# HENDRIX-ZT2/pyaudiorestoration

Measured on AMD Instinct MI355X. Metric: Msamples/sec resampled (192 kHz varispeed), higher is better.
Workload: dtype f32 near taps, far taps (|n| >= 3) as float16 hi + lo x 2^-12 filter banks on v_mfma_f32_16x16x32_f16 with f32 accumulation / f64 positions

## Files before the change

pyaudiorestoration_amd/csrc/pos.hip:

```cpp
#include "par_common.h"
#include "pos_plan.h"
#include <math.h>
#include <vector>

#pragma clang fp contract(off)

namespace par {

struct AddU128 {
  using T = U128;
  __device__ static T identity() { return T{0ull, 0ull}; }
  __device__ static T combine(T a, T b) {
    T r;
    r.lo = a.lo + b.lo;
    r.hi = a.hi + b.hi + (r.lo < a.lo ? 1ull : 0ull);
    return r;
  }
};
struct AddF64 {
  using T = double;
  __device__ static T identity() { return 0.0; }
  __device__ static T combine(T a, T b) { return a + b; }
};
struct ComposeP {
// ... 869 lines not shown
  if (x < n_tiles) {
    const long long start = seg_start[lo], k = sample - start, b = k >> 3;
    static_assert(kCk == 8, "k >> 3");
    const double off = seg_off[lo];
    const bool off_ok = fabs(off) < 4.0e18;
    const double ro = off_ok ? rint(off) : 0.0;
    const long long slot = ck_slot0(start, lo) + b;
    const double ckv = lazy ? (lazy_segment_ok(seg_start[lo + 1] - start, sp[lo], sp[lo + 1])
                                   ? lazy_prefix(sp[lo], (sp[lo + 1] - sp[lo]) / (double)(seg_start[lo + 1] - start - 1), (double)(k + 1))
                                   : 0.0)
                            : ((b && slot < ck_len) ? ck[slot] : 0.0);
    const double rel = (off_ok ? off - ro : 0.0) + ckv;
    const bool ok = off_ok && fabs(rel) < 1.0e15 && ro > -0x1p61 && ro < 0x1p61;
    TileHdr hd;
    hd.anchor = ok ? ((long long)ro + (long long)rint(rel)) & ~1ll : 0ll;
    hd.c_last = 0;
    hd.iT = lo;
    hd.mn_rel = 0;
    bool may_unity = false, may_slow = false;
    for (long long q = lo; q < nseg && seg_start[q] <= sample + kSincTileOutputs; ++q) {
      may_unity = may_unity || !(sp[q] < kUnityHintBelow) || !(sp[q + 1] < kUnityHintBelow);
      may_slow = may_slow || !(sp[q] >= kSlowHintBelow) || !(sp[q + 1] >= kSlowHintBelow);
    }
    hd.flags = (ok ? 0 : 1) | (may_unity ? kTileMayUnity : 0) | (may_slow ? kTileMaySlow : 0) | (lazy ? kTileLazy : 0);
    hdr[x] = hd;
  }
}

__device__ __forceinline__ void tile_seg_body(const double* __restrict__ sp, const int64_t* __restrict__ seg_start,
                           const double* __restrict__ seg_off, int64_t nseg, const double* __restrict__ ck, int64_t ck_len,
                           int64_t max_tiles, int64_t* __restrict__ tile_seg, SegFast* __restrict__ seg_fast,
                           long long* __restrict__ tile_st, TileHdr* __restrict__ hdr, PlanHeader* __restrict__ h, const int64_t x,
                           const bool lazy = false) {
// ... 92 lines not shown
  const double z = rc * step;
  double cprev = ckv;
  if (uk) {
    if (fast) {
      const double x = z * (-0.5 * (double)(uk + 1) - 16.0);
      const double r = rc * __builtin_fma(x, __builtin_fma(x, -x, x) - 1.0, 1.0);
      cprev += r * (double)uk * __builtin_fma(z * z, (double)(uk * uk - 1) * (1.0 / 12.0), 1.0);
    } else {
      for (int v = 0; v < uk; ++v) cprev += recip_nr(__builtin_fma(step, k - (double)(uk - v), s0));
    }
  }
  return piece_poly(foff + cprev, rc, z, -16);
}
__device__ __forceinline__ bool irel_ok(long long rel) { return rel > -32000 && rel < 32000; }

__global__ __launch_bounds__(256) void k_block_rec2(const double* __restrict__ sp, const int64_t* __restrict__ seg_start,
                                                    int64_t nseg, const SegFast* __restrict__ seg_fast,
                                                    const TileHdr* __restrict__ hdr, BlockRec* __restrict__ rec,
                                                    BlockRec2* __restrict__ rec2, const PlanHeader* __restrict__ h) {
  const long long i = (long long)blockIdx.x * blockDim.x + threadIdx.x;
  if (i < 1 || i >= nseg || !h->ck_valid) return;
  const long long start = seg_start[i];
  const int us = (int)(start & (kRec - 1));
  if (us == 0 || start >= h->len_out) return;
  const SegFast s1 = seg_fast[i];
  const double rc = recip_nr(__builtin_fma(s1.step, (double)(16 - us), sp[i]));
  const BlockPoly b1 = piece_poly(s1.foff, rc, rc * s1.step, us - 16);
  const double r1 = rint(b1.a0);
  const long long rel = s1.A + (long long)r1 - hdr[start / kSincTileOutputs].anchor;
  BlockRec2 o2;
  o2.w0 = (unsigned)((int)rel << 16);
  o2.F = (float)(b1.a0 - r1);
  o2.e1 = (float)b1.a1m1;
  o2.e2 = (float)b1.a2;
  rec2[start >> kRecShift] = o2;
  if (!(fabs(b1.a0) < 1.0e9 && irel_ok(rel))) atomicOr(&rec[start >> kRecShift].w0, kRecSlow1);
}

__global__ __launch_bounds__(256) void k_block_rec(const double* __restrict__ sp, const int64_t* __restrict__ seg_start,
                                                   int64_t nseg, const double* __restrict__ ck,
                                                   const int64_t* __restrict__ tile_seg, const long long* __restrict__ tile_st,
                                                   const SegFast* __restrict__ seg_fast, const TileHdr* __restrict__ hdr,
                                                   BlockRec* __restrict__ rec, const PlanHeader* __restrict__ h) {
  const long long len_out = h->len_out;
  if (!h->ck_valid) return;
  const long long g = (long long)blockIdx.x * blockDim.x + threadIdx.x;
  const long long jb = g * kRec;
  if (jb >= len_out) return;
  const long long T = g / kBlocksPerTile;
  const long long j0 = T * kSincTileOutputs;
  const long long iT = tile_seg[T];
  int Sr[kTileStarts];
#pragma unroll
  for (int q = 0; q < kTileStarts; ++q) {
    const long long d = tile_st[T * kTileStarts + q] - j0;
    Sr[q] = d < -0x40000000ll ? -0x40000000 : (d > 0x40000000ll ? 0x40000000 : (int)d);
  }
// ... 60 lines not shown
    end1 = s1.n == need;
    slow1 = !(i + 1 < nseg && s1.fast >= 2 && s1.n >= need && s1.A > -(1ll << 61) && s1.A < (1ll << 61) && sp1 >= 0.971 &&
              sp1 <= 1.031) ||
            (ul >= (long long)ustar && ul < kRec);
    cubic |= s1.fast == 2;
  }
  BlockRec o;
  const bool e0 = (ustar < (unsigned)kRec) || rem == kRec;
  if (end1) slow1 = 1u;
  o.w0 = ((unsigned)((int)rel0 << 16)) | (ustar - 1u) | (e0 ? kRecE0 : 0u) | (end1 ? kRecE1 : 0u) | (slow0 ? kRecSlow0 : 0u) |
         (slow1 ? kRecSlow1 : 0u) | (cubic ? kRecCubic : 0u) | ((e0 ? ustar - 1u : 63u) << kRecLastShift);
  o.F = (float)(q0.a0 - r0);
  o.e1 = (float)q0.a1m1;
  o.e2 = (float)q0.a2;
  rec[g] = o;
}

constexpr int kRecLazySegs = 64;
#ifndef PAR_REC_EXP
#define PAR_REC_EXP 0
#endif
__device__ __forceinline__ double recip_nr_c(double b) {
#pragma clang fp contract(fast)
  double x = __builtin_amdgcn_rcp(b);
  x = x + x * (1.0 - b * x);
  return x + x * (1.0 - b * x);
}
__device__ __forceinline__ BlockPoly piece_poly_c(double base, double rc, double z, int d0) {
#pragma clang fp contract(fast)
  const double rp = -(rc * z), cz = rc * z * z, dd0 = (double)d0;
  const double s2m = (dd0 - 1.0) * dd0 * (2.0 * dd0 - 1.0) * (1.0 / 6.0);
  BlockPoly q;
  q.a0 = ((base + rc * (1.0 - dd0)) + 0.5 * rp * (dd0 - dd0 * dd0)) - cz * s2m;
  q.a1m1 = ((rc - 1.0) + 0.5 * rp) + cz * (1.0 / 6.0);
  q.a2 = 0.5 * rp + 0.5 * cz;
  return q;
}
__device__ __forceinline__ double lazy_prefix_nr(double s0, double step, double K) {
#pragma clang fp contract(fast)
  const double rc = recip_nr_c(__builtin_fma(step, 0.5 * (K - 1.0), s0));
  const double z = rc * step, t = z * z, K2 = K * K;
  return K * rc * (1.0 + t * (K2 - 1.0) * (1.0 / 12.0) * (1.0 + t * (3.0 * K2 - 7.0) * 0.05));
}
__global__ __launch_bounds__(256) void k_block_rec_lazy(const double* __restrict__ sp, const int64_t* __restrict__ seg_start,
                                                        int64_t nseg, const SegFast* __restrict__ seg_fast,
                                                        const TileHdr* __restrict__ hdr, BlockRec* __restrict__ rec,
                                                        BlockRec2* __restrict__ rec2, const PlanHeader* __restrict__ h) {
  __shared__ SegFast s_sf[4][kRecLazySegs + 1];
  __shared__ double s_sp[4][kRecLazySegs + 2];
  __shared__ int s_a[4][kRecLazySegs + 1];
  __shared__ unsigned char s_fl[4][kRecLazySegs];
  __shared__ unsigned char s_seg[4][kRecLazySegs * (kLazyMaxN / kRec)];
  static_assert(kLazyMaxN % kRec == 0 && kRecLazySegs <= 256, "a segment owns <= kLazyMaxN / kRec block starts; indices fit a byte");
  constexpr unsigned kF_Slow1 = 1u, kF_End1 = 2u, kF_Cubic1 = 4u;
  if (h->ck_valid != 2) return;
  const int l = threadIdx.x & (kWave - 1), w = threadIdx.x >> 6;
  const long long i0 = ((long long)blockIdx.x * 4 + w) * kRecLazySegs;
  if (i0 >= nseg) return;
  const long long len_out = h->len_out;
  const long long a0 = seg_start[i0];
  if (a0 >= len_out) return;
// ... 105 lines not shown
    o.F = (float)(q0.a0 - r0);
    o.e1 = (float)q0.a1m1;
    o.e2 = (float)q0.a2;
#if PAR_REC_EXP & 1
    if (o.w0 == 0x12345678u)
#endif
#if PAR_REC_EXP & 4
    {
      typedef unsigned u4v __attribute__((ext_vector_type(4)));
      u4v v = {o.w0, __float_as_uint(o.F), __float_as_uint(o.e1), __float_as_uint(o.e2)};
      __builtin_nontemporal_store(v, reinterpret_cast<u4v*>(rec + g));
    }
#else
    rec[g] = o;
#endif
  }
}

__device__ __forceinline__ void mark_direct(long long i, long long* direct, PlanHeader* h) {
  const int slot = atomicAdd(&h->n_direct, 1);
  if (slot < kMaxDirect) direct[slot] = i;
  else atomicOr(&h->flags, kFlagDirectOverflow);
}

__global__ void k_off_prepare(const double* __restrict__ S, const double* __restrict__ xs, const double* __restrict__ st,
                              int64_t nseg, PElem* __restrict__ el, long long* __restrict__ direct,
                              PlanHeader* __restrict__ h) {
  const int64_t i = (int64_t)blockIdx.x * blockDim.x + threadIdx.x;
  if (i >= nseg) return;
  const double st0 = st[0];
// ... 751 lines not shown
  hipLaunchKernelGGL(k_long_map, dim3(gc), dim3(256), 0, s, speeds, pv.seg_start, nseg, ck, ck_len, G, pv.hdr);
  hipLaunchKernelGGL(k_long_wmap, dim3(gw), dim3(256), 0, s, pv.seg_start, nseg, ck, ck_len, GW, pv.hdr);
  hipLaunchKernelGGL(k_long_stitch, dim3(gs), dim3(256), 0, s, speeds, pv.seg_start, nseg, ck, ck_len, pv.hdr);
  hipLaunchKernelGGL(k_long_wapply, dim3(gw), dim3(256), 0, s, pv.seg_start, nseg, ck, ck_len, GW, pv.hdr);
  hipLaunchKernelGGL(k_long_final, dim3(gc), dim3(256), 0, s, speeds, pv.seg_start, nseg, pv.S, ck, ck_len, G, pv.hdr);
  return PAR_OK;
}

static void launch_block_rec(const double* speeds, const par::PlanView& pv, int64_t nseg, void* aux, int64_t max_out, int64_t m,
                             hipStream_t s) {
  using namespace par;
  const FusedAux a = fused_aux_view(aux, max_out, m);
  const int64_t blocks = (int64_t)fused_blocks(max_out);
  hipLaunchKernelGGL(k_block_rec, dim3((unsigned)ceil_div(blocks, 256)), dim3(256), 0, s, speeds, pv.seg_start, nseg,
                     (const double*)a.ck, (const int64_t*)a.tile_seg, (const long long*)a.tile_st, (const SegFast*)a.seg_fast,
                     (const TileHdr*)a.hdr, a.rec, (const PlanHeader*)pv.hdr);
  hipLaunchKernelGGL(k_block_rec2, dim3((unsigned)ceil_div(nseg, 256)), dim3(256), 0, s, speeds, pv.seg_start, nseg,
                     (const SegFast*)a.seg_fast, (const TileHdr*)a.hdr, a.rec, a.rec2, (const PlanHeader*)pv.hdr);
}

static thread_local int g_last_plan_flags = 0;

static int plan_impl(int device, const double* sampletimes, const double* speeds, int64_t m, int64_t n_in, void* work,
                     size_t work_bytes, void* aux, size_t aux_bytes, int64_t max_out, int64_t* len_out, int* trimmed,
                     int force_host, int* path_used, int* fused_ok, void* stream) {
  using namespace par;
  PAR_REQUIRE(sampletimes && speeds && work && len_out && trimmed, PAR_ERR_ARG, "par_speed_to_pos_plan: null pointer");
  PAR_REQUIRE(m >= 2, PAR_ERR_ARG, "par_speed_to_pos_plan: need at least 2 speed samples (m=%lld)", (long long)m);
  PAR_REQUIRE(work_bytes >= plan_bytes(m), PAR_ERR_WORKSPACE, "par_speed_to_pos_plan: workspace %zu < %zu", work_bytes,
              plan_bytes(m));
  PAR_REQUIRE(!aux || aux_bytes >= fused_aux_bytes(max_out, m), PAR_ERR_WORKSPACE,
              "par_speed_to_pos_plan: aux buffer %zu < %zu", aux_bytes, aux ? fused_aux_bytes(max_out, m) : (size_t)0);
  PAR_HIP_CHECK(hipSetDevice(device));
// ... 54 lines not shown
    hipLaunchKernelGGL(k_off_heads, dim3((kMaxDirect + 255) / 256), dim3(256), 0, s, el, nseg, pv.direct, pv.hdr);
    hipLaunchKernelGGL(k_scan_reduce<ComposeP>, dim3(nbs), dim3(kScanThreads), 0, s, (const PElem*)el, nseg,
                       reinterpret_cast<PElem*>(pv.bsum));
    hipLaunchKernelGGL(k_scan_top<ComposeP>, dim3(1), dim3(kScanThreads), 0, s, reinterpret_cast<PElem*>(pv.bsum), (int64_t)nbs);
    hipLaunchKernelGGL(k_scan_apply<ComposeP>, dim3(nbs), dim3(kScanThreads), 0, s, el, nseg, (const PElem*)pv.bsum);
    hipLaunchKernelGGL(k_off_stitch, dim3(1), dim3(1), 0, s, pv.S, el, sampletimes, nseg, pv.direct, pv.runs, pv.hdr);
    if (lazy) {
      hipLaunchKernelGGL(k_off_apply, dim3(g256), dim3(256), 0, s, speeds, (const PElem*)el, (const RunEntry*)pv.runs, nseg,
                         (double)n_in, pv.seg_off, pv.hdr);
      hipLaunchKernelGGL(k_trim_lazy, dim3(1), dim3(1), 0, s, sampletimes, speeds, (const int64_t*)pv.seg_start,
                         (const double*)pv.seg_off, m, (double)n_in, ck_len, max_tiles, pv.hdr);
      const FusedAux av = fused_aux_view(aux, max_out, m);
      hipLaunchKernelGGL(k_tile_seg_lazy, dim3(g256), dim3(256), 0, s, speeds, (const int64_t*)pv.seg_start,
                         (const double*)pv.seg_off, nseg, av.tile_seg, av.seg_fast, av.tile_st, av.hdr, (const PlanHeader*)pv.hdr);
      hipLaunchKernelGGL(k_block_rec_lazy, dim3((unsigned)ceil_div(nseg, 4 * kRecLazySegs)), dim3(256), 0, s, speeds, (const int64_t*)pv.seg_start, nseg,
                         (const SegFast*)av.seg_fast, (const TileHdr*)av.hdr, av.rec, av.rec2, (const PlanHeader*)pv.hdr);
    } else {
    hipLaunchKernelGGL(k_off_apply_trim, dim3(g256 < 512u ? g256 : 512u), dim3(256), 0, s, sampletimes, speeds, (const PElem*)el,
                       (const RunEntry*)pv.runs, (const int64_t*)pv.seg_start, nseg, (double)n_in, pv.seg_off,
                       (const double*)ck, ck_len, pv.hdr);
    }
    if (aux && !lazy) {
      const int64_t n_items = std::max<int64_t>(nseg, max_tiles);
      hipLaunchKernelGGL(k_tile_seg_publish, dim3((unsigned)std::min<int64_t>(ceil_div(n_items, 256), 512)), dim3(256), 0, s,
                         speeds, pv.seg_start, pv.seg_off, nseg, (const double*)ck, ck_len, max_tiles,
                         reinterpret_cast<int64_t*>(ck + ck_len), reinterpret_cast<SegFast*>(ck + ck_len + max_tiles),
                         fused_aux_view(aux, max_out, m).tile_st, fused_aux_view(aux, max_out, m).hdr, pv.hdr, n_items,
                         lazy ? 1 : 0);
      launch_block_rec(speeds, pv, nseg, aux, max_out, m, s);
    }
    PAR_HIP_CHECK(hipGetLastError());
// ... 110 lines not shown
```

pyaudiorestoration_amd/csrc/pos_plan.h:

```cpp
#pragma once
#include "par_common.h"

namespace par {

struct PlanHeader {
  int64_t m;
  int64_t len_out;
  int64_t total_written;
  unsigned long long trim_seg;
  int64_t cap;
  int32_t trimmed;
  int32_t flags;
  int32_t n_direct;
  int32_t n_runs;
  double speed_sum;
  int64_t ck_len;
  int32_t ck_valid;
  int32_t pad2;
  int64_t written;
  int32_t n_long;
  int32_t pad3;
  unsigned long long first_bad;
  int32_t lazy;
  int32_t lazy_fail;
// ... 141 lines not shown
  int fast;
};
static_assert(sizeof(SegFast) == 32, "SegFast is loaded as two 16-byte words");
constexpr int kRec = 32;
constexpr int kRecShift = 5;
struct BlockRec {
  unsigned w0;
  float F, e1, e2;
};
static_assert(sizeof(BlockRec) == 16, "BlockRec is one 16-byte word");
constexpr int kRecLastShift = 10;
constexpr unsigned kRecE0 = 1u << 5, kRecE1 = 1u << 6, kRecSlow0 = 1u << 7, kRecSlow1 = 1u << 8, kRecCubic = 1u << 9;
typedef BlockRec BlockRec2;
struct TileHdr {
  long long anchor;
  long long c_last;
  long long iT;
  int mn_rel;
  int flags;
};
constexpr int kTileMayUnity = 2;
constexpr int kTileMaySlow = 8;
constexpr double kSlowHintBelow = 1.0000002;
constexpr double kUnityHintBelow = 0.9999998;
static_assert(sizeof(TileHdr) == 32, "TileHdr is one s_load_dwordx8");
constexpr int kBlocksPerTile = (int)(kSincTileOutputs / kRec);
constexpr int kTileStarts = 6;
inline size_t fused_ck_len(int64_t max_out, int64_t m) { return (size_t)(max_out / kCk + m + 16); }
inline size_t fused_tiles(int64_t max_out) { return (size_t)(max_out / kSincTileOutputs + 4); }
inline size_t fused_blocks(int64_t max_out) { return fused_tiles(max_out) * kBlocksPerTile; }
inline size_t fused_aux_bytes(int64_t max_out, int64_t m) {
  return (fused_ck_len(max_out, m) + fused_tiles(max_out)) * 8 + (size_t)m * sizeof(SegFast) +
         fused_tiles(max_out) * (sizeof(TileHdr) + kTileStarts * 8) +
// ... 29 lines not shown
```

pyaudiorestoration_amd/csrc/sinc2.hip:

```cpp
#define PAR_WANT_BANK2 1
#include "par_common.h"
#include "pos_plan.h"
#include "sinc_taps_gen.h"
#include "sinc_common.h"
#include "sinc_block.h"
#include <algorithm>
#include <atomic>
#include <limits.h>
#include <type_traits>

constexpr int kMaxTilesPerWave = 23;
#ifndef PAR_S2_EXP
#define PAR_S2_EXP 0
#endif

namespace par {

typedef _Float16 half8v __attribute__((ext_vector_type(8)));
typedef _Float16 half2v __attribute__((ext_vector_type(2)));
typedef float float4v __attribute__((ext_vector_type(4)));

constexpr int kRing = 512;
constexpr int kPass = 128;
constexpr float kImgScale = 1024.0f, kImgScaleInv = 0.0009765625f;
// ... 24 lines not shown
  int* redo_count;
  int* redo_list;
  int tiles;
  int tiles_tail;
  int64_t n_big;
  int64_t n_full;
  int64_t n_tiles;
  int n_edge;
  int64_t out_stride;
  FusedArgs fa;
  const float4* tab;
  TapModes tmd;
};
constexpr int kEdgeWaveOut = 128;
constexpr int kEdgeWavesPerTile = kSincTileOutputs / kEdgeWaveOut;
constexpr int kTileEdge = 0x100;

__device__ __forceinline__ float sinpi_poly(float z) {
  float p = -0.00737043094f;
  p = fmaf(p, z, 0.0821458866f);
  p = fmaf(p, z, -0.599264529f);
  p = fmaf(p, z, 2.55016404f);
  p = fmaf(p, z, -5.16771278f);
  return fmaf(p, z, 3.14159265f);
}

__device__ __forceinline__ _Float16 hi16(float x) { return (_Float16)(fabsf(x) < 6.103515625e-05f ? 0.0f : x); }
#define S2_HI(x) hi16(x)

__device__ __forceinline__ unsigned pack_h2(float a, float b) {
  const half2v h = {(_Float16)a, (_Float16)b};
// ... 31 lines not shown
               ::"v"(lane_bytes), "s"(bs), "s"(__builtin_amdgcn_readfirstlane(la)) : "memory", "m0");
}

__device__ __forceinline__ void wave_lds_fence() {
  __builtin_amdgcn_fence(__ATOMIC_RELEASE, "wavefront");
  __builtin_amdgcn_wave_barrier();
  __builtin_amdgcn_fence(__ATOMIC_ACQUIRE, "wavefront");
}

__device__ __forceinline__ int clamp64(int n) { return n < 0 ? 0 : (n > 64 ? 64 : n); }
__device__ __forceinline__ unsigned long long prefix(int n) { return n >= 64 ? ~0ull : ((1ull << n) - 1ull); }

struct S2Row {
  int c;
  float s, ep;
  bool bad;
};
template <bool SECOND = true>
__device__ __forceinline__ S2Row s2_place_row(const uint4 ra, const uint4 rb, const int u, const int cbase, const float uf,
                                              const float u2f, const float tw1, const float tw0, const float tolf) {
  const unsigned m = ra.x;
  const bool second = SECOND && (unsigned)u > (m & 31u);
  const float F = __uint_as_float(second ? rb.y : ra.y), e1 = __uint_as_float(second ? rb.z : ra.z),
              e2 = __uint_as_float(second ? rb.w : ra.w);
  const int irel = (int)(second ? rb.x : ra.x) >> 16;
  const bool last = (unsigned)u == ((m >> kRecLastShift) & 63u);
  const float frac = fmaf(u2f, e2, fmaf(uf, e1, F));
  const float e = fmaf(e2, last ? tw0 : tw1, e1);
  const float ri = rintf(frac);
  S2Row o;
  o.s = frac - ri;
  o.c = cbase + irel + (int)ri;
  o.ep = __builtin_amdgcn_fmed3f(e, 0.0f, 3.0e38f);
  o.bad = (m & (kRecSlow0 | kRecSlow1 | kRecCubic)) != 0u || !(fabsf(fabsf(o.s) - 0.5f) > tolf);
  return o;
}


constexpr int kRingF = 1024;
constexpr int kRingH = 512;

template <int NCH, bool MOM = true>
struct S3Lds {
  static constexpr bool kMoments = MOM;
  float ring_head[4 * NCH];
  float ring[kRingF * NCH];
  float ring_tail[4 * NCH];
  _Float16 img[2 * NCH][kRingH];
  float4v qa[kPass];
  float4v qm0[MOM ? kPass : kPass / 4];
  float4v qm1[MOM ? kPass : 1];
  __device__ __forceinline__ float& e2d2(int sl) {
    return MOM ? reinterpret_cast<float*>(&qm0[sl])[3] : reinterpret_cast<float*>(&qm0[0])[sl];
  }
  __device__ __forceinline__ const float& e2d2(int sl) const {
    return MOM ? reinterpret_cast<const float*>(&qm0[sl])[3] : reinterpret_cast<const float*>(&qm0[0])[sl];
  }
#ifdef PAR_S3_LDS_PAD
  uint4 pad[PAR_S3_LDS_PAD / 16];
#endif
  uint4 recs[4][16];
};
static_assert(offsetof(S3Lds<1>, img) % 16 == 0 && offsetof(S3Lds<1>, qa) % 16 == 0 && offsetof(S3Lds<1>, recs) % 16 == 0, "16-byte aligned");
static_assert(offsetof(S3Lds<2>, ring) % 16 == 0 && offsetof(S3Lds<2>, img) % 16 == 0 && offsetof(S3Lds<2>, qa) % 16 == 0 &&
              offsetof(S3Lds<2>, recs) % 16 == 0, "16-byte aligned");
static_assert(sizeof(S3Lds<2>) <= 20480, "eight stereo streams per compute unit (160 KB of LDS)");
using S3LdsUnity = S3Lds<1, false>;
static_assert(sizeof(S3LdsUnity) <= 10240 && offsetof(S3LdsUnity, recs) % 16 == 0 && offsetof(S3LdsUnity, qa) % 16 == 0,
              "sixteen fc = 1 streams per compute unit");

struct S3Pass {
  int c[2];
  float s[2], ep[2];
  int nok[2];
  int j, ws;
};
// ... 199 lines not shown
      fused_wave<NCH, 32, 2 * NCH, true>(a.len_out, a.sig, a.sig + 1, NCH, a.len_in, 32, a.tab, a.tmd, a.out, a.out + 1, NCH, a.fa, piece, l,
                                         jw, nrem, piece);
    else if (nrem > 0)
      fused_wave<NCH, 32, 2 * NCH, false>(a.len_out, a.sig, a.sig + 1, NCH, a.len_in, 32, a.tab, a.tmd, a.out, a.out + 1, NCH, a.fa, piece, l,
                                          jw, nrem, piece);
    return;
    }
  }
  const int64_t stream_id = (int64_t)bx - a.n_edge;
  const int my_tiles = stream_id < a.n_big ? a.tiles : a.tiles_tail;
  const int64_t Ta = stream_id < a.n_big ? stream_id * a.tiles : a.n_big * a.tiles + (stream_id - a.n_big) * a.tiles_tail;
  if (Ta >= a.n_full) return;
  const int64_t Tb = Ta + my_tiles < a.n_full ? Ta + my_tiles : a.n_full;
  const int64_t Ja = Ta * kSincTileOutputs, Jb = Tb * kSincTileOutputs;
  long long A0;
  int hd_dA, hd_fl;
  {
    const int64_t Ti = Ta + l < a.n_tiles ? Ta + l : a.n_tiles - 1;
    const TileHdr h = a.hdr[l <= my_tiles ? Ti : Ta];
    A0 = (long long)(((unsigned long long)(unsigned)__builtin_amdgcn_readfirstlane((int)((unsigned long long)h.anchor >> 32)) << 32) |
                     (unsigned)__builtin_amdgcn_readfirstlane((int)(unsigned)(unsigned long long)h.anchor));
    const long long d = h.anchor - A0;
    hd_fl = h.flags | ((d > -0x40000000ll && d < 0x40000000ll) ? 0 : 1);
    if (a.n_edge > 0 && (Ta + l == 0 || Ta + l >= a.n_full - 2)) hd_fl |= 1 | kTileEdge;
    hd_dA = (int)d;
    if constexpr (KIND == 1 || KIND == 2) {
      const bool any_slow = __ballot(l < my_tiles && Ta + l < Tb && (h.flags & kTileMaySlow) != 0) != 0ull;
      if (any_slow != (KIND == 2)) return;
    }
  }
  half8v fr[kBank2Frags];
  {
    const uint4* src = reinterpret_cast<const uint4*>(kBank2Frags32) + l;
#pragma unroll
    for (int f = 0; f < kBank2Frags; ++f) fr[f] = __builtin_bit_cast(half8v, src[f * kWave]);
  }
  half8v fmr[kBank3Frags];
  if constexpr (kMom) {
    const uint4* src = reinterpret_cast<const uint4*>(kBank3Frags32) + l;
#pragma unroll
// ... 38 lines not shown
    if constexpr (NCH == 2) dma_chunk256(src, lane_bytes, &L.ring[(k & 7) * (kPass * 2)]);
    else dma_chunk128(src, lane_bytes, &L.ring[(k & 7) * kPass]);
  };
  auto push_tile = [&](int64_t T) {
    if (l == 0) {
      const int slot = atomicAdd(a.redo_count, 1);
      a.redo_list[slot] = (int)T;
    }
  };
  if (stream_id == 0 && a.n_full < a.n_tiles && a.n_edge == 0) push_tile(a.n_full);

  struct Placed {
    S2Row R[2];
    int nt[2];
    int fl0, fl1, tend;
    int epm;
  };
  int tc_T = -1, tc_dA0 = 0, tc_dA1 = 0, tc_fl0 = 0, tc_fl1 = 0;
  auto place = [&](int j, int buf, int rb) {
    Placed P;
    const int T = j >> 10;
    P.tend = (T + 1) << 10;
    if (T != tc_T) {
      tc_T = T;
      tc_dA0 = __builtin_amdgcn_readlane(hd_dA, T);
      tc_dA1 = __builtin_amdgcn_readlane(hd_dA, T + 1);
      tc_fl0 = __builtin_amdgcn_readlane(hd_fl, T);
      tc_fl1 = __builtin_amdgcn_readlane(hd_fl, T + 1);
    }
    const int dA0 = tc_dA0, dA1 = tc_dA1;
    P.fl0 = tc_fl0;
    P.fl1 = tc_fl1;
    const int t5 = (j & (kRec - 1)) + l;
    const int u = t5 & (kRec - 1);
    const int bi = ((j >> kRecShift) - rb + (t5 >> kRecShift)) & 7;
    const uint4* rp = &L.recs[buf][0];
    const uint4 ra0 = rp[bi], rb0 = rp[8 + bi], ra1 = rp[(bi + 2) & 7], rb1 = rp[8 + ((bi + 2) & 7)];
    const int uc = u - kRec / 2;
    const float uf = (float)uc, u2f = uf * uf, tw1 = fmaf(2.0f, uf, 1.0f), tw0 = tw1 - 2.0f;
    P.nt[0] = clamp64(P.tend - j);
    P.nt[1] = clamp64(P.tend - j - 64);
    if (__ballot((unsigned)u > (ra0.x & 31u) || (unsigned)u > (ra1.x & 31u)) == 0ull) {
      P.R[0] = s2_place_row<false>(ra0, rb0, u, (l < P.nt[0] ? dA0 : dA1) + uc, uf, u2f, tw1, tw0, tolf);
      P.R[1] = s2_place_row<false>(ra1, rb1, u, (l < P.nt[1] ? dA0 : dA1) + uc, uf, u2f, tw1, tw0, tolf);
    } else {
      P.R[0] = s2_place_row(ra0, rb0, u, (l < P.nt[0] ? dA0 : dA1) + uc, uf, u2f, tw1, tw0, tolf);
      P.R[1] = s2_place_row(ra1, rb1, u, (l < P.nt[1] ? dA0 : dA1) + uc, uf, u2f, tw1, tw0, tolf);
    }
    P.epm = max(__float_as_int(P.R[0].ep), __float_as_int(P.R[1].ep));
    return P;
  };

  S3Pass P;
  P.nok[0] = P.nok[1] = 0;
  P.j = P.ws = 0;
  P.c[0] = P.c[1] = 0;
  P.s[0] = P.s[1] = P.ep[0] = P.ep[1] = 0.0f;

  auto out_pass = [&](auto mode_tag, const S3Pass& Q, float (&res)[2], const int ch = 0) {
    constexpr int MODE = decltype(mode_tag)::value;
    const int wsK = Q.ws - wbase;
#pragma unroll
    for (int r = 0; r < 2; ++r) {
      int ci = Q.c[r] - Q.ws;
      ci = ci < 0 ? 0 : (ci > kPass - 1 ? kPass - 1 : ci);
      float sr = Q.s[r], epr = Q.ep[r];
// ... 35 lines not shown
#define S3_COUNT(k) do { } while (0)
#endif
  auto start_run = [&]() -> bool {
    for (;;) {
      if (j0 >= nJ) return false;
      S3_COUNT(1);
      __builtin_amdgcn_s_waitcnt(0x0F70);
      wave_lds_fence();
      const int buf = pk & 3;
      fetch_records(buf, j0 >> kRecShift);
      __builtin_amdgcn_s_waitcnt(0x0F70);
      wave_lds_fence();
      const Placed Q = place(j0, buf, j0 >> kRecShift);
      const int tend = Q.tend;
      int nv[2] = {clamp64(nJ - j0), clamp64(nJ - j0 - 64)};
      const unsigned long long b0 = __ballot(Q.R[0].bad || !(Q.R[0].ep <= kEpMaxMom)) & prefix(nv[0]),
                               b1 = __ballot(Q.R[1].bad || !(Q.R[1].ep <= kEpMaxMom)) & prefix(nv[1]);
      const unsigned long long bad_here = (b0 & prefix(Q.nt[0])) | (b1 & prefix(Q.nt[1]));
      const bool bad_next = ((b0 & ~prefix(Q.nt[0])) | (b1 & ~prefix(Q.nt[1])) | (unsigned long long)((Q.fl1 & 1) && tend < nJ)) != 0ull;
      if (bad_next) {
        nv[0] = nv[0] < Q.nt[0] ? nv[0] : Q.nt[0];
        nv[1] = nv[1] < Q.nt[1] ? nv[1] : Q.nt[1];
      }
      bool skip = (Q.fl0 & 1) || bad_here != 0ull;
      const unsigned long long gen = (__ballot(1.0f + Q.R[0].ep != 1.0f) & prefix(nv[0])) | (__ballot(1.0f + Q.R[1].ep != 1.0f) & prefix(nv[1]));
      const int ws = __builtin_amdgcn_readfirstlane(Q.R[0].c) & ~7;
      S3Pass N;
#pragma unroll
      for (int r = 0; r < 2; ++r) {
        N.c[r] = Q.R[r].c;
        N.s[r] = Q.R[r].s;
        N.ep[r] = Q.R[r].ep;
        const unsigned long long in = __ballot(Q.R[r].c - ws < kPass);
        N.nok[r] = __popcll(in & prefix(nv[r]));
// ... 116 lines not shown
      if constexpr (NCH == 2) asm volatile("s_waitcnt vmcnt(7)" ::: "memory");
      else asm volatile("s_waitcnt vmcnt(5)" ::: "memory");
#if PAR_S2_EXP & 64
      const unsigned long long tB_ = __builtin_readcyclecounter();
      s3t_[0] += tB_ - tA_;
      s3t_[1] += tA_ - s3last_;
      s3last_ = tB_;
      s3t_[2] += 1;
#endif
      wave_lds_fence();
      S3Pass N;
      bool ok;
      int wsK;
      auto place_next = [&]() {
      const Placed Q = place(j0, pk & 3, rbA);
      const unsigned long long bad = __ballot(Q.R[0].bad || Q.R[1].bad || Q.epm > __float_as_int(kEpMaxMom));
      const unsigned long long gen = __ballot(Q.epm > 0x33800000);
      bool tier = true;
      if constexpr (MODE == 2) tier = __ballot(Q.epm > __float_as_int(kEpMom5)) == 0ull;
      if constexpr (MODE == 3) tier = __ballot(Q.epm > __float_as_int(kEpMom5Lo)) != 0ull;
      const int ws = __builtin_amdgcn_readfirstlane(Q.R[0].c) & ~7;
#pragma unroll
      for (int r = 0; r < 2; ++r) {
        N.c[r] = Q.R[r].c;
        N.s[r] = Q.R[r].s;
        N.ep[r] = Q.R[r].ep;
        N.nok[r] = __popcll(__ballot(Q.R[r].c - ws < kPass));
      }
      N.j = j0;
      N.ws = ws;
      wsK = ws - wbase;
      const int d = kPass * conv_next - wsK;
      ok = (((Q.fl0 | Q.fl1) & 1) == 0) & (bad == 0ull) & (j0 + kPass <= nJ) & (N.nok[0] + N.nok[1] >= 120) &
           (MODE == 1 ? gen == 0ull : gen != 0ull) & tier & ((unsigned)(d - 161) <= 312u) & (conv_next + 1 < dma_bad) &
           ((unsigned)((j0 >> kRecShift) - rbA) <= 1u);
      };
      if constexpr (!kTwo) place_next();
      float res[2];
      out_pass(mode_tag, P, res);
      bool cok;
      if constexpr (kTwo) {
        float res1[2];
        asm volatile("" : "+v"(res[0]), "+v"(res[1]));
        bank_image3m<MODE != 1, MODE == 3>(L, fr, fmr, P.ws - wbase - 31, l, 1);
        out_pass(mode_tag, P, res1, 1);
        asm volatile("" : "+v"(res1[0]), "+v"(res1[1]));
        place_next();
        const int offs = wsK - 31;
// ... 10 lines not shown
        asm volatile("" : "+v"(res[0]), "+v"(res[1]));
#endif
        bank_image3m<MODE != 1, MODE == 3>(L, fr, fmr, offs, l);
        cok = convert_chunk(conv_next);
        fetch_records((pk + 2) & 3, rbC);
        chunk_dma(dma_next);
        store_pass(P, res);
      }
      wave_lds_fence();
      ++conv_next;
      ++dma_next;
      if (!cok) mode = 0;
      S3_COUNT(2);
#if PAR_S2_EXP & 128
      if (!(ok && cok)) {
        if (((Q.fl0 | Q.fl1) & 1) != 0 || bad != 0ull) S3_COUNT(3);
        else if (!(j0 + kPass <= nJ)) S3_COUNT(4);
        else if (!(N.nok[1] >= 1 && N.nok[0] + N.nok[1] >= 120)) S3_COUNT(5);
        else if (!(MODE == 1 ? gen == 0ull : gen != 0ull)) S3_COUNT(6);
        else if (!(d >= 161 && d <= 473)) S3_COUNT(7);
        else if (!(conv_next < dma_bad)) S3_COUNT(9);
        else if (!((unsigned)((j0 >> kRecShift) - rbA) <= 1u)) S3_COUNT(11);
        else if (!cok) S3_COUNT(10);
        else S3_COUNT(8);
      }
#endif
      if (!(ok && cok)) {
        if constexpr (kTwo)
          if (mode != 0 && !s3_convert_ch(L, conv_next - 1, l, 1, false)) mode = 0;
        return;
      }
// ... 145 lines not shown
```

Before: 170,200.

## Precompute per-tile block end/bad bitmasks to simplify sinc placement path

Planning kernels now build per-tile 32-bit bitmasks of block-end and slow/cubic blocks using wave ballots and atomicOr into the tile header. The sinc stage loads these masks into LDS and uses them to pick a cheaper single-record placement path, and to flag bad blocks without reading the second record or per-lane flag bits. Momentum/error-bound work is compiled out when kMom is off. This adds atomics in the planning kernels and changes the flag packing (tighter anchor delta range, flags packed with the delta), which could push more tiles onto the slow path.

```diff
diff --git a/pyaudiorestoration_amd/csrc/pos.hip b/pyaudiorestoration_amd/csrc/pos.hip
--- a/pyaudiorestoration_amd/csrc/pos.hip
+++ b/pyaudiorestoration_amd/csrc/pos.hip
@@ -907,9 +907,9 @@
     const bool ok = off_ok && fabs(rel) < 1.0e15 && ro > -0x1p61 && ro < 0x1p61;
     TileHdr hd;
     hd.anchor = ok ? ((long long)ro + (long long)rint(rel)) & ~1ll : 0ll;
-    hd.c_last = 0;
+    hd.m_end = hd.m_bad = 0u;
+    hd.pad = 0;
     hd.iT = lo;
-    hd.mn_rel = 0;
     bool may_unity = false, may_slow = false;
     for (long long q = lo; q < nseg && seg_start[q] <= sample + kSincTileOutputs; ++q) {
       may_unity = may_unity || !(sp[q] < kUnityHintBelow) || !(sp[q + 1] < kUnityHintBelow);
@@ -1032,9 +1032,24 @@
 }
 __device__ __forceinline__ bool irel_ok(long long rel) { return rel > -32000 && rel < 32000; }
 
+__device__ __forceinline__ void tile_masks_or(TileHdr* hdr, long long g0, bool end, bool bad) {
+  const unsigned long long be = __ballot(end), bb = __ballot(bad);
+  const int l = threadIdx.x & (kWave - 1);
+  if (l >= 3) return;
+  const int sh = (int)(g0 & (kBlocksPerTile - 1));
+  static_assert(kBlocksPerTile == 32, "a 32-bit mask per tile");
+  auto word = [&](unsigned long long B) -> unsigned {
+    return (unsigned)(l == 0 ? B << sh : (l == 1 ? B >> (32 - sh) : (sh ? B >> (64 - sh) : 0ull)));
+  };
+  TileHdr* const t = hdr + (g0 >> 5) + l;
+  const unsigned we = word(be), wb = word(bb);
+  if (we) atomicOr(&t->m_end, we);
+  if (wb) atomicOr(&t->m_bad, wb);
+}
+
 __global__ __launch_bounds__(256) void k_block_rec2(const double* __restrict__ sp, const int64_t* __restrict__ seg_start,
                                                     int64_t nseg, const SegFast* __restrict__ seg_fast,
-                                                    const TileHdr* __restrict__ hdr, BlockRec* __restrict__ rec,
+                                                    TileHdr* hdr, BlockRec* __restrict__ rec,
                                                     BlockRec2* __restrict__ rec2, const PlanHeader* __restrict__ h) {
   const long long i = (long long)blockIdx.x * blockDim.x + threadIdx.x;
   if (i < 1 || i >= nseg || !h->ck_valid) return;
@@ -1052,13 +1067,16 @@
   o2.e1 = (float)b1.a1m1;
   o2.e2 = (float)b1.a2;
   rec2[start >> kRecShift] = o2;
-  if (!(fabs(b1.a0) < 1.0e9 && irel_ok(rel))) atomicOr(&rec[start >> kRecShift].w0, kRecSlow1);
+  if (!(fabs(b1.a0) < 1.0e9 && irel_ok(rel))) {
+    atomicOr(&rec[start >> kRecShift].w0, kRecSlow1);
+    atomicOr(&hdr[start / kSincTileOutputs].m_bad, 1u << ((start >> kRecShift) & (kBlocksPerTile - 1)));
+  }
 }
 
 __global__ __launch_bounds__(256) void k_block_rec(const double* __restrict__ sp, const int64_t* __restrict__ seg_start,
                                                    int64_t nseg, const double* __restrict__ ck,
                                                    const int64_t* __restrict__ tile_seg, const long long* __restrict__ tile_st,
-                                                   const SegFast* __restrict__ seg_fast, const TileHdr* __restrict__ hdr,
+                                                   const SegFast* __restrict__ seg_fast, TileHdr* hdr,
                                                    BlockRec* __restrict__ rec, const PlanHeader* __restrict__ h) {
   const long long len_out = h->len_out;
   if (!h->ck_valid) return;
@@ -1149,6 +1167,7 @@
   o.e1 = (float)q0.a1m1;
   o.e2 = (float)q0.a2;
   rec[g] = o;
+  tile_masks_or(hdr, g - (threadIdx.x & (kWave - 1)), e0, slow0 || slow1 || cubic);
 }
 
 constexpr int kRecLazySegs = 64;
@@ -1179,7 +1198,7 @@
 }
 __global__ __launch_bounds__(256) void k_block_rec_lazy(const double* __restrict__ sp, const int64_t* __restrict__ seg_start,
                                                         int64_t nseg, const SegFast* __restrict__ seg_fast,
-                                                        const TileHdr* __restrict__ hdr, BlockRec* __restrict__ rec,
+                                                        TileHdr* hdr, BlockRec* __restrict__ rec,
                                                         BlockRec2* __restrict__ rec2, const PlanHeader* __restrict__ h) {
   __shared__ SegFast s_sf[4][kRecLazySegs + 1];
   __shared__ double s_sp[4][kRecLazySegs + 2];
@@ -1315,6 +1334,7 @@
 #else
     rec[g] = o;
 #endif
+    tile_masks_or(hdr, g - l, e0, slow0 || slow1 || cubic);
   }
 }
 
@@ -2096,9 +2116,9 @@
   const int64_t blocks = (int64_t)fused_blocks(max_out);
   hipLaunchKernelGGL(k_block_rec, dim3((unsigned)ceil_div(blocks, 256)), dim3(256), 0, s, speeds, pv.seg_start, nseg,
                      (const double*)a.ck, (const int64_t*)a.tile_seg, (const long long*)a.tile_st, (const SegFast*)a.seg_fast,
-                     (const TileHdr*)a.hdr, a.rec, (const PlanHeader*)pv.hdr);
+                     a.hdr, a.rec, (const PlanHeader*)pv.hdr);
   hipLaunchKernelGGL(k_block_rec2, dim3((unsigned)ceil_div(nseg, 256)), dim3(256), 0, s, speeds, pv.seg_start, nseg,
-                     (const SegFast*)a.seg_fast, (const TileHdr*)a.hdr, a.rec, a.rec2, (const PlanHeader*)pv.hdr);
+                     (const SegFast*)a.seg_fast, a.hdr, a.rec, a.rec2, (const PlanHeader*)pv.hdr);
 }
 
 static thread_local int g_last_plan_flags = 0;
@@ -2183,7 +2203,7 @@
       hipLaunchKernelGGL(k_tile_seg_lazy, dim3(g256), dim3(256), 0, s, speeds, (const int64_t*)pv.seg_start,
                          (const double*)pv.seg_off, nseg, av.tile_seg, av.seg_fast, av.tile_st, av.hdr, (const PlanHeader*)pv.hdr);
       hipLaunchKernelGGL(k_block_rec_lazy, dim3((unsigned)ceil_div(nseg, 4 * kRecLazySegs)), dim3(256), 0, s, speeds, (const int64_t*)pv.seg_start, nseg,
-                         (const SegFast*)av.seg_fast, (const TileHdr*)av.hdr, av.rec, av.rec2, (const PlanHeader*)pv.hdr);
+                         (const SegFast*)av.seg_fast, av.hdr, av.rec, av.rec2, (const PlanHeader*)pv.hdr);
     } else {
     hipLaunchKernelGGL(k_off_apply_trim, dim3(g256 < 512u ? g256 : 512u), dim3(256), 0, s, sampletimes, speeds, (const PElem*)el,
                        (const RunEntry*)pv.runs, (const int64_t*)pv.seg_start, nseg, (double)n_in, pv.seg_off,
diff --git a/pyaudiorestoration_amd/csrc/pos_plan.h b/pyaudiorestoration_amd/csrc/pos_plan.h
--- a/pyaudiorestoration_amd/csrc/pos_plan.h
+++ b/pyaudiorestoration_amd/csrc/pos_plan.h
@@ -179,9 +179,10 @@
 typedef BlockRec BlockRec2;
 struct TileHdr {
   long long anchor;
-  long long c_last;
+  unsigned m_end;
+  unsigned m_bad;
   long long iT;
-  int mn_rel;
+  int pad;
   int flags;
 };
 constexpr int kTileMayUnity = 2;
diff --git a/pyaudiorestoration_amd/csrc/sinc2.hip b/pyaudiorestoration_amd/csrc/sinc2.hip
--- a/pyaudiorestoration_amd/csrc/sinc2.hip
+++ b/pyaudiorestoration_amd/csrc/sinc2.hip
@@ -62,7 +62,9 @@
 };
 constexpr int kEdgeWaveOut = 128;
 constexpr int kEdgeWavesPerTile = kSincTileOutputs / kEdgeWaveOut;
-constexpr int kTileEdge = 0x100;
+constexpr int kTilePush = 1;
+constexpr int kTileEdge = 2;
+constexpr int kTileBad = 4;
 
 __device__ __forceinline__ float sinpi_poly(float z) {
   float p = -0.00737043094f;
@@ -124,25 +126,39 @@
 struct S2Row {
   int c;
   float s, ep;
-  bool bad;
+  bool tie;
 };
-template <bool SECOND = true>
+__device__ __forceinline__ bool s2_tie(const float s, const float tolf) { return !(fabsf(fabsf(s) - 0.5f) > tolf); }
+template <bool EP>
+__device__ __forceinline__ S2Row s2_place_plain(const uint4 ra, const int cbase, const float uf, const float u2f, const float tw1) {
+  const float F = __uint_as_float(ra.y), e1 = __uint_as_float(ra.z), e2 = __uint_as_float(ra.w);
+  const float frac = fmaf(u2f, e2, fmaf(uf, e1, F));
+  const float ri = rintf(frac);
+  S2Row o;
+  o.s = frac - ri;
+  o.c = cbase + ((int)ra.x >> 16) + (int)ri;
+  o.ep = EP ? __builtin_amdgcn_fmed3f(fmaf(e2, tw1, e1), 0.0f, 3.0e38f) : 0.0f;
+  return o;
+}
+template <bool EP>
 __device__ __forceinline__ S2Row s2_place_row(const uint4 ra, const uint4 rb, const int u, const int cbase, const float uf,
-                                              const float u2f, const float tw1, const float tw0, const float tolf) {
+                                              const float u2f, const float tw1, const float tw0) {
   const unsigned m = ra.x;
-  const bool second = SECOND && (unsigned)u > (m & 31u);
+  const bool second = (unsigned)u > (m & 31u);
   const float F = __uint_as_float(second ? rb.y : ra.y), e1 = __uint_as_float(second ? rb.z : ra.z),
               e2 = __uint_as_float(second ? rb.w : ra.w);
   const int irel = (int)(second ? rb.x : ra.x) >> 16;
-  const bool last = (unsigned)u == ((m >> kRecLastShift) & 63u);
   const float frac = fmaf(u2f, e2, fmaf(uf, e1, F));
-  const float e = fmaf(e2, last ? tw0 : tw1, e1);
   const float ri = rintf(frac);
   S2Row o;
   o.s = frac - ri;
   o.c = cbase + irel + (int)ri;
-  o.ep = __builtin_amdgcn_fmed3f(e, 0.0f, 3.0e38f);
-  o.bad = (m & (kRecSlow0 | kRecSlow1 | kRecCubic)) != 0u || !(fabsf(fabsf(o.s) - 0.5f) > tolf);
+  o.ep = 0.0f;
+  if constexpr (EP) {
+    const bool last = (unsigned)u == ((m >> kRecLastShift) & 63u);
+    const float e = fmaf(e2, last ? tw0 : tw1, e1);
+    o.ep = __builtin_amdgcn_fmed3f(e, 0.0f, 3.0e38f);
+  }
   return o;
 }
 
@@ -170,6 +186,7 @@
   uint4 pad[PAR_S3_LDS_PAD / 16];
 #endif
   uint4 recs[4][16];
+  uint2 tmask[48];
 };
 static_assert(offsetof(S3Lds<1>, img) % 16 == 0 && offsetof(S3Lds<1>, qa) % 16 == 0 && offsetof(S3Lds<1>, recs) % 16 == 0, "16-byte aligned");
 static_assert(offsetof(S3Lds<2>, ring) % 16 == 0 && offsetof(S3Lds<2>, img) % 16 == 0 && offsetof(S3Lds<2>, qa) % 16 == 0 &&
@@ -399,16 +416,20 @@
   const int64_t Tb = Ta + my_tiles < a.n_full ? Ta + my_tiles : a.n_full;
   const int64_t Ja = Ta * kSincTileOutputs, Jb = Tb * kSincTileOutputs;
   long long A0;
-  int hd_dA, hd_fl;
+  int hd_dA;
   {
     const int64_t Ti = Ta + l < a.n_tiles ? Ta + l : a.n_tiles - 1;
     const TileHdr h = a.hdr[l <= my_tiles ? Ti : Ta];
     A0 = (long long)(((unsigned long long)(unsigned)__builtin_amdgcn_readfirstlane((int)((unsigned long long)h.anchor >> 32)) << 32) |
                      (unsigned)__builtin_amdgcn_readfirstlane((int)(unsigned)(unsigned long long)h.anchor));
     const long long d = h.anchor - A0;
-    hd_fl = h.flags | ((d > -0x40000000ll && d < 0x40000000ll) ? 0 : 1);
-    if (a.n_edge > 0 && (Ta + l == 0 || Ta + l >= a.n_full - 2)) hd_fl |= 1 | kTileEdge;
-    hd_dA = (int)d;
+    const bool d_ok = d > -0x10000000ll && d < 0x10000000ll;
+    int hd_fl = (h.flags & 1) | (d_ok ? 0 : kTilePush);
+    if (a.n_edge > 0 && (Ta + l == 0 || Ta + l >= a.n_full - 2)) hd_fl |= kTilePush | kTileEdge;
+    if (l <= my_tiles) L.tmask[l] = make_uint2(h.m_end, h.m_bad);
+    if (h.m_bad) hd_fl |= kTileBad;
+    if (KIND == 1 && l < my_tiles && (h.flags & kTileMaySlow)) hd_fl |= kTilePush;
+    hd_dA = (int)((unsigned)(d_ok ? (int)d : 0) << 3) | hd_fl;
     if constexpr (KIND == 1 || KIND == 2) {
       const bool any_slow = __ballot(l < my_tiles && Ta + l < Tb && (h.flags & kTileMaySlow) != 0) != 0ull;
       if (any_slow != (KIND == 2)) return;
@@ -477,42 +498,59 @@
     S2Row R[2];
     int nt[2];
     int fl0, fl1, tend;
+    unsigned bad;
     int epm;
   };
   int tc_T = -1, tc_dA0 = 0, tc_dA1 = 0, tc_fl0 = 0, tc_fl1 = 0;
+  unsigned long long tc_m = 0, tc_bad = 0;
   auto place = [&](int j, int buf, int rb) {
     Placed P;
     const int T = j >> 10;
     P.tend = (T + 1) << 10;
     if (T != tc_T) {
       tc_T = T;
-      tc_dA0 = __builtin_amdgcn_readlane(hd_dA, T);
-      tc_dA1 = __builtin_amdgcn_readlane(hd_dA, T + 1);
-      tc_fl0 = __builtin_amdgcn_readlane(hd_fl, T);
-      tc_fl1 = __builtin_amdgcn_readlane(hd_fl, T + 1);
+      const int h0 = __builtin_amdgcn_readlane(hd_dA, T), h1 = __builtin_amdgcn_readlane(hd_dA, T + 1);
+      tc_dA0 = h0 >> 3;
+      tc_dA1 = h1 >> 3;
+      tc_fl0 = h0 & 7;
+      tc_fl1 = h1 & 7;
+      const uint2 m0 = L.tmask[T], m1 = L.tmask[T + 1];
+      tc_m = (unsigned)__builtin_amdgcn_readfirstlane((int)m0.x) |
+             ((unsigned long long)(unsigned)__builtin_amdgcn_readfirstlane((int)m1.x) << 32);
+      tc_bad = 0ull;
+      if ((tc_fl0 | tc_fl1) & kTileBad)
+        tc_bad = (unsigned)__builtin_amdgcn_readfirstlane((int)m0.y) |
+                 ((unsigned long long)(unsigned)__builtin_amdgcn_readfirstlane((int)m1.y) << 32);
     }
     const int dA0 = tc_dA0, dA1 = tc_dA1;
     P.fl0 = tc_fl0;
     P.fl1 = tc_fl1;
+    const int sb = (j >> kRecShift) & (kBlocksPerTile - 1);
+    const unsigned mw = (unsigned)(tc_m >> sb);
+    P.bad = (unsigned)(tc_bad >> sb) & 31u;
     const int t5 = (j & (kRec - 1)) + l;
     const int u = t5 & (kRec - 1);
     const int bi = ((j >> kRecShift) - rb + (t5 >> kRecShift)) & 7;
     const uint4* rp = &L.recs[buf][0];
-    const uint4 ra0 = rp[bi], rb0 = rp[8 + bi], ra1 = rp[(bi + 2) & 7], rb1 = rp[8 + ((bi + 2) & 7)];
     const int uc = u - kRec / 2;
-    const float uf = (float)uc, u2f = uf * uf, tw1 = fmaf(2.0f, uf, 1.0f), tw0 = tw1 - 2.0f;
+    const float uf = (float)uc, u2f = uf * uf, tw1 = fmaf(2.0f, uf, 1.0f);
     P.nt[0] = clamp64(P.tend - j);
     P.nt[1] = clamp64(P.tend - j - 64);
-    if (__ballot((unsigned)u > (ra0.x & 31u) || (unsigned)u > (ra1.x & 31u)) == 0ull) {
-      P.R[0] = s2_place_row<false>(ra0, rb0, u, (l < P.nt[0] ? dA0 : dA1) + uc, uf, u2f, tw1, tw0, tolf);
-      P.R[1] = s2_place_row<false>(ra1, rb1, u, (l < P.nt[1] ? dA0 : dA1) + uc, uf, u2f, tw1, tw0, tolf);
+    const int jt = __builtin_amdgcn_readfirstlane(P.tend - j);
+    const uint4 ra0 = rp[bi], ra1 = rp[(bi + 2) & 7];
+    if ((mw & ((j & (kRec - 1)) ? 31u : 15u)) == 0u && jt >= kPass) {
+      P.R[0] = s2_place_plain<kMom>(ra0, dA0 + uc, uf, u2f, tw1);
+      P.R[1] = s2_place_plain<kMom>(ra1, dA0 + uc, uf, u2f, tw1);
     } else {
-      P.R[0] = s2_place_row(ra0, rb0, u, (l < P.nt[0] ? dA0 : dA1) + uc, uf, u2f, tw1, tw0, tolf);
-      P.R[1] = s2_place_row(ra1, rb1, u, (l < P.nt[1] ? dA0 : dA1) + uc, uf, u2f, tw1, tw0, tolf);
-    }
-    P.epm = max(__float_as_int(P.R[0].ep), __float_as_int(P.R[1].ep));
+      P.R[0] = s2_place_row<kMom>(ra0, rp[8 + bi], u, (l < P.nt[0] ? dA0 : dA1) + uc, uf, u2f, tw1, tw1 - 2.0f);
+      P.R[1] = s2_place_row<kMom>(ra1, rp[8 + ((bi + 2) & 7)], u, (l < P.nt[1] ? dA0 : dA1) + uc, uf, u2f, tw1, tw1 - 2.0f);
+    }
+    P.R[0].tie = s2_tie(P.R[0].s, tolf);
+    P.R[1].tie = s2_tie(P.R[1].s, tolf);
+    P.epm = kMom ? max(__float_as_int(P.R[0].ep), __float_as_int(P.R[1].ep)) : 0;
     return P;
   };
+  auto blocks_of = [](int j, int n) -> unsigned { return n > 0 ? (2u << (((j & (kRec - 1)) + n - 1) >> kRecShift)) - 1u : 0u; };
 
   S3Pass P;
   P.nok[0] = P.nok[1] = 0;
@@ -578,10 +616,13 @@
       const Placed Q = place(j0, buf, j0 >> kRecShift);
       const int tend = Q.tend;
       int nv[2] = {clamp64(nJ - j0), clamp64(nJ - j0 - 64)};
-      const unsigned long long b0 = __ballot(Q.R[0].bad || !(Q.R[0].ep <= kEpMaxMom)) & prefix(nv[0]),
-                               b1 = __ballot(Q.R[1].bad || !(Q.R[1].ep <= kEpMaxMom)) & prefix(nv[1]);
-      const unsigned long long bad_here = (b0 & prefix(Q.nt[0])) | (b1 & prefix(Q.nt[1]));
-      const bool bad_next = ((b0 & ~prefix(Q.nt[0])) | (b1 & ~prefix(Q.nt[1])) | (unsigned long long)((Q.fl1 & 1) && tend < nJ)) != 0ull;
+      const unsigned long long b0 = __ballot(Q.R[0].tie || !(Q.R[0].ep <= kEpMaxMom)) & prefix(nv[0]),
+                               b1 = __ballot(Q.R[1].tie || !(Q.R[1].ep <= kEpMaxMom)) & prefix(nv[1]);
+      const int nvt = nv[0] + nv[1], nin = nvt < tend - j0 ? nvt : tend - j0;
+      const unsigned blk_here = blocks_of(j0, nin), blk_all = blocks_of(j0, nvt);
+      const unsigned long long bad_here = (b0 & prefix(Q.nt[0])) | (b1 & prefix(Q.nt[1])) | (Q.bad & blk_here);
+      const bool bad_next = ((b0 & ~prefix(Q.nt[0])) | (b1 & ~prefix(Q.nt[1])) | (Q.bad & blk_all & ~blk_here) |
+                             (unsigned long long)((Q.fl1 & 1) && tend < nJ)) != 0ull;
       if (bad_next) {
         nv[0] = nv[0] < Q.nt[0] ? nv[0] : Q.nt[0];
         nv[1] = nv[1] < Q.nt[1] ? nv[1] : Q.nt[1];
@@ -728,7 +769,8 @@
       int wsK;
       auto place_next = [&]() {
       const Placed Q = place(j0, pk & 3, rbA);
-      const unsigned long long bad = __ballot(Q.R[0].bad || Q.R[1].bad || Q.epm > __float_as_int(kEpMaxMom));
+      const bool bad = (Q.bad & ((j0 & (kRec - 1)) ? 31u : 15u)) != 0u ||
+                       (__ballot(Q.R[0].tie) | __ballot(Q.R[1].tie) | __ballot(kMom && Q.epm > __float_as_int(kEpMaxMom))) != 0ull;
       const unsigned long long gen = __ballot(Q.epm > 0x33800000);
       bool tier = true;
       if constexpr (MODE == 2) tier = __ballot(Q.epm > __float_as_int(kEpMom5)) == 0ull;
@@ -745,7 +787,7 @@
       N.ws = ws;
       wsK = ws - wbase;
       const int d = kPass * conv_next - wsK;
-      ok = (((Q.fl0 | Q.fl1) & 1) == 0) & (bad == 0ull) & (j0 + kPass <= nJ) & (N.nok[0] + N.nok[1] >= 120) &
+      ok = (((Q.fl0 | Q.fl1) & 1) == 0) & !bad & (j0 + kPass <= nJ) & (N.nok[0] + N.nok[1] >= 120) &
            (MODE == 1 ? gen == 0ull : gen != 0ull) & tier & ((unsigned)(d - 161) <= 312u) & (conv_next + 1 < dma_bad) &
            ((unsigned)((j0 >> kRecShift) - rbA) <= 1u);
       };
@@ -786,7 +828,7 @@
       S3_COUNT(2);
 #if PAR_S2_EXP & 128
       if (!(ok && cok)) {
-        if (((Q.fl0 | Q.fl1) & 1) != 0 || bad != 0ull) S3_COUNT(3);
+        if (((Q.fl0 | Q.fl1) & 1) != 0 || bad) S3_COUNT(3);
         else if (!(j0 + kPass <= nJ)) S3_COUNT(4);
         else if (!(N.nok[1] >= 1 && N.nok[0] + N.nok[1] >= 120)) S3_COUNT(5);
         else if (!(MODE == 1 ? gen == 0ull : gen != 0ull)) S3_COUNT(6);
```

Result: no change. 170,700 (median of 6 runs) (+0.3%).
